# Tamnemng/TAM-GCN

Hardware: AMD Instinct MI355X
Metric: skeleton clips/sec (fwd+CE+bwd+grad all-reduce+SGD step), N-UCLA 20-joint x 64-frame (higher is better)
Workload: dtype f32 (exact fp32-input MFMA v_mfma_f32_16x16x4_f32 in every GEMM, forward and backward: the reference's arithmetic); 1 GPU; N-UCLA joint stream, 256 clips/GPU x (3,64,20,1), models.ctrgcn.Model fwd+CE+bwd+grad-allreduce+SGD step, train-mode BN; global_batch=256, streams=1, parallelism=dp1, launch=hipgraph, model_streams=0, rehearsal=False, allreduce=one flat bucket after backward

## Files before the change

include/tamgcn.h:

```cpp
#ifndef TAMGCN_H
#define TAMGCN_H

#ifdef __cplusplus
extern "C" {
#endif

#define TAMGCN_VERSION 401
#define TAMGCN_MAX_SUBSETS 3
#define TAMGCN_MAX_V 32

typedef struct tamgcn_src {
    const float* x1;
    const float* x2;
    const float* coef;
    int ctot;
    int coff;
    int act;
} tamgcn_src;

int         tamgcn_version(void);
const char* tamgcn_last_error(void);
const char* tamgcn_last_kernel(void);
int         tamgcn_get_split_mode(void);
int         tamgcn_set_split_mode(int mode);
// ... 86 lines not shown
    const float* pq;
    const float* w3;
    const float* b3;
    const float* w4;
    const float* b4;
    const float* A;
    const float* alpha;
    const float* E;
} tamgcn_ctrgc_desc;

int tamgcn_ctrgc_build_e(const tamgcn_ctrgc_desc* d, float* E, void* stream);

int tamgcn_ctrgc_fwd(const tamgcn_ctrgc_desc* d, float* y, float* stats_part, float* x3_out, void* stream);

int tamgcn_ctrgc_bwd_dx3(const tamgcn_ctrgc_desc* d, const tamgcn_src* dy,
                         float* dx3, float* db3_part, void* stream);

int tamgcn_ctrgc_bwd_de_acc(const tamgcn_ctrgc_desc* d, const tamgcn_src* dy, const float* x3,
                            float* dE, void* stream);
int tamgcn_ctrgc_bwd_de_tail(const tamgcn_ctrgc_desc* d, const float* dE,
                             float* dA_part, float* dw4_part, float* db4_part,
                             float* dalpha_part, float* dpq, int groups, void* stream);

int tamgcn_ctrgc_tiled_supported(int V);
int tamgcn_ctrgc_tiled_chunks(int V);
int tamgcn_ctrgc_tiled_build_e(const tamgcn_ctrgc_desc* d, float* E, void* stream);
int tamgcn_ctrgc_tiled_agg_fwd(const tamgcn_ctrgc_desc* d, const float* x3, const float* E, float* y, float* stats_part, void* stream);
int tamgcn_ctrgc_tiled_agg_bwd(const tamgcn_ctrgc_desc* d, const tamgcn_src* dy, const float* E, float* dx3, float* db3_part, void* stream);
int tamgcn_ctrgc_tiled_de_acc(const tamgcn_ctrgc_desc* d, const tamgcn_src* dy, const float* x3, float* dE, void* stream);
int tamgcn_ctrgc_tiled_de_tail(const tamgcn_ctrgc_desc* d, const float* dE, float* dA_part, float* dw4_part, float* db4_part,
                               float* dalpha_part, float* dpq, void* stream);

int tamgcn_vgen_supported(int V);
int tamgcn_vgen_lds_bytes(int S, int V, int R);
int tamgcn_vgen_build_e(const tamgcn_ctrgc_desc* d, float* E, void* stream);
int tamgcn_vgen_agg_fwd(const tamgcn_ctrgc_desc* d, const float* x3, const float* E, float* y, float* stats_part, void* stream);
int tamgcn_vgen_agg_bwd(const tamgcn_ctrgc_desc* d, const tamgcn_src* dy, const float* E, float* dx3, float* db3_part, void* stream);
int tamgcn_vgen_de_acc(const tamgcn_ctrgc_desc* d, const tamgcn_src* dy, const float* x3, float* dE, void* stream);
int tamgcn_vgen_de_tail(const tamgcn_ctrgc_desc* d, const float* dE, float* dA_part, float* dw4_part, float* db4_part,
                        float* dalpha_part, float* dpq, int groups, void* stream);

int tamgcn_ew_nparts(int N, int C, int T, int V);

int tamgcn_gcn_tail_fwd(const tamgcn_src* y, const tamgcn_src* o, const tamgcn_src* res,
                        int N, int C, int T, int V, float* g, void* stream);
int tamgcn_gcn_tail_bwd(const float* dg, const float* g, const tamgcn_src* o, const float* o_save,
// ... 156 lines not shown
```

tam_gcn_amd/_lib.py:

```python
import ctypes as C
import os

_HERE = os.path.dirname(os.path.abspath(__file__))
LIB_PATH = os.path.join(_HERE, 'libtamgcn.so')

c_float_p = C.c_void_p


class Src(C.Structure):
    _fields_ = [('x1', C.c_void_p), ('x2', C.c_void_p), ('coef', C.c_void_p),
                ('ctot', C.c_int), ('coff', C.c_int), ('act', C.c_int)]


class ConvDesc(C.Structure):
    _fields_ = [('src', Src),
                ('N', C.c_int), ('K', C.c_int), ('T_in', C.c_int), ('V', C.c_int),
                ('w', C.c_void_p), ('bias', C.c_void_p),
                ('M', C.c_int), ('KT', C.c_int), ('dil', C.c_int), ('stride', C.c_int), ('pad', C.c_int),
                ('wmode', C.c_int), ('up', C.c_int),
                ('y', C.c_void_p), ('yctot', C.c_int), ('ycoff', C.c_int),
                ('T_out', C.c_int), ('T_y', C.c_int), ('ostride', C.c_int),
                ('add1', C.c_void_p), ('add2', C.c_void_p), ('bcast', C.c_void_p), ('bcast_scale', C.c_float),
                ('mask', C.POINTER(Src)),
                ('aux', C.c_void_p), ('aux_center', C.c_void_p), ('auxctot', C.c_int), ('auxcoff', C.c_int),
# ... 91 lines not shown
    'tamgcn_conv_nparts': (_i, [C.POINTER(ConvDesc)]),
    'tamgcn_conv': (_i, [C.POINTER(ConvDesc), _p]),
    'tamgcn_wgrad_max_split': (_i, [C.POINTER(WgradDesc)]),
    'tamgcn_wgrad': (_i, [C.POINTER(WgradDesc), _p]),
    'tamgcn_stem_stats': (_i, [_p, _p, _p, _i, _i, _i, _i, _i, _p, _p]),
    'tamgcn_stem_apply': (_i, [_p, _p, _p, _i, _i, _i, _i, _i, _p, _p]),
    'tamgcn_head_pool_fwd': (_i, [_p, _i, _i, _i, _i, _i, _p, _p]),
    'tamgcn_head_pool_bwd': (_i, [_p, _i, _i, _i, _i, _i, _p, _p]),
    'tamgcn_head_fc_fwd': (_i, [_p, _p, _p, _i, _i, _i, _p, _p]),
    'tamgcn_head_fc_bwd': (_i, [_p, _p, _p, _i, _i, _i, _p, _p, _p, _p]),
    'tamgcn_reduce_multi': (_i, [C.POINTER(ReduceDesc), _i, _p]),
    'tamgcn_reduce_sum': (_i, [_p, _i, _ll, _ll, _f, _i, _p, _p]),
    'tamgcn_bn_fwd_finalize': (_i, [_p, _i, _i, _i, _d, _p, _p, _p, _p, _p, _f, _f, _i, _p, _p, _i, _i, _i, _p]),
    'tamgcn_bn_bwd_finalize': (_i, [_p, _i, _i, _i, _d, _p, _p, _i, _i, _i, _p, _p, _p, _p, _i, _i, _i, _p]),
    'tamgcn_bn_fwd_finalize_multi': (_i, [C.POINTER(BnFwdDesc), _i, _p]),
    'tamgcn_coef_diff': (_i, [_p, _p, _p, _i, _i, _p]),
    'tamgcn_bn_bwd_finalize_multi': (_i, [C.POINTER(BnBwdDesc), _i, _p]),
    'tamgcn_tmean': (_i, [_SP, _i, _i, _i, _i, _p, _p]),
    'tamgcn_ctrgc_build_e': (_i, [C.POINTER(CtrgcDesc), _p, _p]),
    'tamgcn_ctrgc_fwd': (_i, [C.POINTER(CtrgcDesc), _p, _p, _p, _p]),
    'tamgcn_ctrgc_bwd_dx3': (_i, [C.POINTER(CtrgcDesc), _SP, _p, _p, _p]),
    'tamgcn_ctrgc_bwd_de_acc': (_i, [C.POINTER(CtrgcDesc), _SP, _p, _p, _p]),
    'tamgcn_ctrgc_bwd_de_tail': (_i, [C.POINTER(CtrgcDesc), _p, _p, _p, _p, _p, _p, _i, _p]),
    'tamgcn_ctrgc_tiled_supported': (_i, [_i]),
    'tamgcn_ctrgc_tiled_chunks': (_i, [_i]),
    'tamgcn_ctrgc_tiled_build_e': (_i, [C.POINTER(CtrgcDesc), _p, _p]),
    'tamgcn_ctrgc_tiled_agg_fwd': (_i, [C.POINTER(CtrgcDesc), _p, _p, _p, _p, _p]),
    'tamgcn_ctrgc_tiled_agg_bwd': (_i, [C.POINTER(CtrgcDesc), _SP, _p, _p, _p, _p]),
    'tamgcn_ctrgc_tiled_de_acc': (_i, [C.POINTER(CtrgcDesc), _SP, _p, _p, _p]),
    'tamgcn_ctrgc_tiled_de_tail': (_i, [C.POINTER(CtrgcDesc), _p, _p, _p, _p, _p, _p, _p]),
    'tamgcn_vgen_supported': (_i, [_i]),
    'tamgcn_vgen_lds_bytes': (_i, [_i, _i, _i]),
    'tamgcn_vgen_build_e': (_i, [C.POINTER(CtrgcDesc), _p, _p]),
    'tamgcn_vgen_agg_fwd': (_i, [C.POINTER(CtrgcDesc), _p, _p, _p, _p, _p]),
    'tamgcn_vgen_agg_bwd': (_i, [C.POINTER(CtrgcDesc), _SP, _p, _p, _p, _p]),
    'tamgcn_vgen_de_acc': (_i, [C.POINTER(CtrgcDesc), _SP, _p, _p, _p]),
    'tamgcn_vgen_de_tail': (_i, [C.POINTER(CtrgcDesc), _p, _p, _p, _p, _p, _p, _i, _p]),
    'tamgcn_ew_nparts': (_i, [_i, _i, _i, _i]),
    'tamgcn_gcn_tail_fwd': (_i, [_SP, _SP, _SP, _i, _i, _i, _i, _p, _p]),
    'tamgcn_gcn_tail_bwd': (_i, [_p, _p, _SP, _p, _i, _i, _i, _i, _p, _p, _p, _p]),
    'tamgcn_gcn_mid_bwd': (_i, [_p, _p, _p, _p, _p, _p, _i, _i, _i, _i, _p, _p, _p, _p]),
    'tamgcn_tconv_supported': (_i, [_i, _i, _i, _i, C.POINTER(C.c_int), _i, _i]),
    'tamgcn_tconv_nparts': (_i, [C.POINTER(TconvDesc), _i]),
    'tamgcn_tconv_fwd': (_i, [C.POINTER(TconvDesc), _p]),
    'tamgcn_tconv_bwd': (_i, [C.POINTER(TconvDesc), _p]),
    'tamgcn_tconv_wgrad_max_split': (_i, [C.POINTER(TconvDesc)]),
# ... 79 lines not shown
```

tam_gcn_amd/build.py:

```python
import os
import subprocess
import sys

HERE = os.path.dirname(os.path.abspath(__file__))
SRC = ['lib.hip', 'conv.hip', 'wgrad.hip', 'reduce.hip', 'bn.hip', 'elementwise.hip', 'ctrgc.hip', 'ctrgc_de.hip', 'ctrgc_tiled.hip', 'vgen.hip', 'stemhead.hip', 'feeder.hip', 'f2.hip', 'f2v.hip', 'tconv.hip', 'optim.hip', 'evalmeter.hip']
LIB = os.path.join(HERE, 'libtamgcn.so')
ARCH = 'gfx950'


def _hipcc():
    for c in (os.environ.get('HIPCC'), '/opt/rocm/bin/hipcc', 'hipcc'):
        if c and (os.path.isabs(c) and os.path.exists(c) or not os.path.isabs(c)):
            return c
    return 'hipcc'


def sources():
    return [os.path.join(HERE, 'csrc', s) for s in SRC]


def needs_build():
    if not os.path.exists(LIB):
        return True
    deps = sources() + [os.path.join(HERE, 'csrc', 'common.h'), os.path.join(HERE, 'csrc', 'evalbody.h'),
                        os.path.join(HERE, '..', 'include', 'tamgcn.h')]
    t = os.path.getmtime(LIB)
    return any(os.path.getmtime(d) > t for d in deps)

# ... 28 lines not shown
```

tam_gcn_amd/csrc/ctrgc.hip:

```cpp
#include "common.h"
#include <stdlib.h>

TG_TRACE_DEFINE(tamgcn_trace_read_ctrgc)

#ifndef TG_CKO
#define TG_CKO 0
#endif

namespace {

struct CtrgcArgs {
    int N, Cin, Cout, S, T;
    const float* x; int x_ctot, x_coff;
    const float* w3; const float* b3;
    const float* E;
    int nct;
};

template <int V_, int CT_, int TB_, int NTQ_, int SBK_>
struct Geo {
    static constexpr int V = V_, CT = CT_, TB = TB_, NTQ = NTQ_, SBK = SBK_;
    static constexpr int SBKP = SBK + 2;
    static constexpr int NT = CT * NTQ * 4;
    static constexpr int NW = NT / 64;
// ... 143 lines not shown
                for (int k = 0; k < 8; ++k)
                    if (k * 4 < a.R) acc = mfma16(aw[k], Ds[(k * 4 + kq) * VV + colc], acc);
                if (col < VV) {
#pragma unroll
                    for (int r = 0; r < 4; ++r) Eg[(long long)(c0 + kq * 4 + r) * VV + col] = alpha * (acc[r] + b4r[r]) + Ar[it];
                }
            }
        }
        if (c0 + 16 < a.Cout) {
#pragma unroll
            for (int k = 0; k < 8; ++k) aw[k] = awn[k];
#pragma unroll
            for (int r = 0; r < 4; ++r) b4r[r] = b4n[r];
        }
    }
}

template <class G, int ST, bool UL = false>
struct X3Pref {
    using P = Plan<G, ST>;
    static constexpr int NPF = G::NPF, NT = G::NT, SBK = G::SBK, CT = G::CT;
    static constexpr int ROWV = G::NCOLS / 4;
    static constexpr int NAF = (P::NRT * 16 * SBK + NT - 1) / NT;
    float4 rv[NPF];
    float wv[NAF];

    __device__ __forceinline__ void load(const CtrgcArgs& a, int n, int c0, int t0, int bt, int k0, int tid) {
        if (TG_CKO & 2) return;
        constexpr int V = G::V;
        const int ncols = bt * V;
        const int cs = a.T * V;
        const float* xk = a.x + ((long long)n * a.x_ctot + a.x_coff + k0) * cs + (long long)t0 * V;
        const float* wk = a.w3 + (long long)c0 * a.Cin + k0;
        if constexpr (UL) {
            xk = a.x + cg_sgpr(((long long)n * a.x_ctot + a.x_coff + k0) * cs + (long long)t0 * V);
            wk = a.w3 + cg_sgpr((long long)c0 * a.Cin + k0);
        }
#pragma unroll
        for (int i = 0; i < NAF; ++i) {
            const int e = tid + i * NT;
            const int kk = e % SBK, row = e / SBK;
            const int sidx = row / CT, c = row - sidx * CT;
            const bool ok = row < P::NR && k0 + kk < a.Cin;
            if constexpr (UL) wv[i] = *cg_at<float>(wk, ok ? 4u * (unsigned)((sidx * a.Cout + c) * a.Cin + kk) : 0u);
            else wv[i] = ok ? *cg_at<float>(wk, 4u * (unsigned)((sidx * a.Cout + c) * a.Cin + kk)) : 0.f;
        }
#pragma unroll
        for (int i = 0; i < NPF; ++i) {
            const int e = tid + i * NT;
            const int kk = e / ROWV, pos = (e - kk * ROWV) * 4;
            const bool ok = kk < SBK && k0 + kk < a.Cin && pos < ncols;
            if constexpr (UL) rv[i] = *cg_at<float4>(xk, ok ? 4u * (unsigned)(kk * cs + pos) : 0u);
            else rv[i] = ok ? *cg_at<float4>(xk, 4u * (unsigned)(kk * cs + pos)) : make_float4(0.f, 0.f, 0.f, 0.f);
        }
    }
    __device__ __forceinline__ void pin() {
#pragma unroll
        for (int i = 0; i < NPF; ++i) asm volatile("" : "+v"(rv[i].x), "+v"(rv[i].y), "+v"(rv[i].z), "+v"(rv[i].w));
#pragma unroll
        for (int i = 0; i < NAF; ++i) asm volatile("" : "+v"(wv[i]));
    }
    __device__ __forceinline__ void commit(float* As, float* Bs, int tid, int Cin, int k0, int ncols) const {
        if (TG_CKO & 4) return;
#pragma unroll
        for (int i = 0; i < NAF; ++i) {
            const int e = tid + i * NT;
            const int kk = e % SBK, row = e / SBK;
            if constexpr (UL) {
                if (row < P::NRT * 16) As[row * G::SBKP + kk] = (row < P::NR && k0 + kk < Cin) ? wv[i] : 0.f;
            } else {
                if (row < P::NRT * 16) As[row * G::SBKP + kk] = wv[i];
            }
        }
#pragma unroll
        for (int i = 0; i < NPF; ++i) {
            const int e = tid + i * NT;
            const int kk = e / ROWV, pos = (e - kk * ROWV) * 4;
            if constexpr (UL) {
                if (kk < SBK) *reinterpret_cast<float4*>(Bs + kk * G::PITCHB + pos) = (k0 + kk < Cin && pos < ncols) ? rv[i] : make_float4(0.f, 0.f, 0.f, 0.f);
            } else {
                if (kk < SBK) *reinterpret_cast<float4*>(Bs + kk * G::PITCHB + pos) = rv[i];
            }
        }
    }
};

template <class G, int ST, bool UL, class Pre>
__device__ __forceinline__ void x3_chunk(const CtrgcArgs& a, int n, int c0, int t0, int bt, float* X3, X3Pref<G, ST, UL>& pf, int next_t0, int next_bt, int tid, Pre&& pre, float* B3s = nullptr, float b3v = 0.f) {
    using P = Plan<G, ST>;
    constexpr int V = G::V, CW = G::CW, SBK = G::SBK, SBKP = G::SBKP, CT = G::CT;
    constexpr int NR = P::NR, NRT = P::NRT, PB = G::PITCHB;
    const int lane = tid & 63, wave = tid >> 6;
    const int j = lane & 15, kq = lane >> 4;
    const int ncols = bt * V;
    constexpr bool BAL = (G::NW == 8 && G::NCT == 20);
    const int cw0 = BAL ? 5 * (wave & 3) + (wave < 4 ? 0 : 3) : wave * CW;
    const bool third = !BAL || wave < 4;
    float* Bs = X3;
    float* As = X3 + SBK * PB;

    f32x4 acc[NRT][CW];
#pragma unroll
// ... 36 lines not shown
#pragma unroll
                for (int rt = 0; rt < NRT; ++rt) asm volatile("" : "=v"(av[rt]));
#pragma unroll
                for (int c = 0; c < CW; ++c) asm volatile("" : "=v"(bv[c]));
            } else {
#pragma unroll
            for (int rt = 0; rt < NRT; ++rt) av[rt] = at[rt * 16 * SBKP + k4 * 4];
#pragma unroll
            for (int c = 0; c < CW; ++c) bv[c] = bt_[k4 * 4 * PB + bcol[c]];
            }
            if ((TG_CKO & 1) && k4) continue;
#pragma unroll
            for (int c = 0; c < (BAL ? 2 : CW); ++c)
#pragma unroll
                for (int rt = 0; rt < NRT; ++rt) acc[rt][c] = mfma16(av[rt], bv[c], acc[rt][c]);
            if (BAL && third) {
#pragma unroll
                for (int rt = 0; rt < NRT; ++rt) acc[rt][2] = mfma16(av[rt], bv[2], acc[rt][2]);
            }
        }
    }
    pre();
    __syncthreads();
#pragma unroll
    for (int rt = 0; rt < NRT; ++rt) {
        if constexpr (UL) {
            const f32x4 b = *reinterpret_cast<const f32x4*>(B3s + rt * 16 + kq * 4);
#pragma unroll
            for (int r = 0; r < 4; ++r) b3r[rt][r] = b[r];
        }
#pragma unroll
        for (int c = 0; c < CW; ++c) {
            int col = (cw0 + c) * 16 + j;
            if ((TG_CKO & 8) && (rt || c)) continue;
            if (col >= ncols || (BAL && c == 2 && !third)) continue;
            const int fr = col / V, v = col - fr * V;
#pragma unroll
            for (int r = 0; r < 4; ++r) {
                const int row = rt * 16 + kq * 4 + r;
                const int sidx = row / CT, ch = row - sidx * CT;
                if (row < NR) X3[(ch * G::BT + fr) * (ST * V) + sidx * V + v] = acc[rt][c][r] + b3r[rt][r];
            }
        }
    }
    __syncthreads();
}
// ... 195 lines not shown
        const int lrow = tid % (G::NTQ * 4);
        TG_T(ta);
        EFrag<G, ST> ef;
        x3_chunk<G, ST, !ER>(a, n, c0, t0, bt, X3, pf, nt0, nbt, tid, [&] { if constexpr (!ER) ef.ld(En, a.Cout, c0 + __builtin_amdgcn_readfirstlane(tid >> 6), tid); }, Zs, b3v);
        TG_T(tb); TG_ACC(1, tb - ta);
        if constexpr (!ER) aggregate_mfma_g<G, ST>(En, a.Cout, c0, ef, X3, Zs, bt, tid);
        else if (!(TG_CKO & 16)) aggregate_mfma<G, ST>(Es, X3, Zs, bt);
        TG_T(tc); TG_ACC(2, tc - tb);
        __syncthreads();
        TG_T(td); TG_ACC(3, td - tc);
        constexpr int RL = G::NTQ * 4;
        constexpr int NV4 = (G::NCOLS / 4 + RL - 1) / RL;
        float* ybase = y + (((long long)n * a.Cout + c0) * a.T + t0) * V;
        const unsigned rowb = 4u * (unsigned)(c * a.T * V);
        float4 zv[NV4];
#pragma unroll
        for (int i = 0; i < NV4; ++i) {
            const int p4 = lrow + i * RL;
            zv[i] = p4 < (ncols >> 2) ? reinterpret_cast<const float4*>(Zs + c * G::NCOLS)[p4] : make_float4(0.f, 0.f, 0.f, 0.f);
        }
        if (nbt > 0) pf.pin();
        if constexpr (!ER) {
            if (x3_out) {
#pragma unroll
                for (int s = 0; s < ST; ++s) {
                    float4 xs[NV4];
#pragma unroll
                    for (int i = 0; i < NV4; ++i) {
                        const int p4 = lrow + i * RL;
                        const int fr = p4 / (V / 4), q = p4 - fr * (V / 4);
                        xs[i] = p4 < (ncols >> 2) ? *reinterpret_cast<const float4*>(X3 + (c * G::BT + fr) * (ST * V) + s * V + 4 * q)
                                                  : make_float4(0.f, 0.f, 0.f, 0.f);
                    }
                    float* xo = x3_out + (((long long)n * ST * a.Cout + s * a.Cout + c0) * a.T + t0) * V;
#pragma unroll
                    for (int i = 0; i < NV4; ++i) {
                        const int p4 = lrow + i * RL;
                        if (p4 < (ncols >> 2)) *cg_at_w<float4>(xo, rowb + 16u * (unsigned)p4) = xs[i];
                    }
                }
            }
        } else
        if (x3_out) {
            float4 xv[ST][NV4];
#pragma unroll
            for (int s = 0; s < ST; ++s)
#pragma unroll
                for (int i = 0; i < NV4; ++i) {
                    const int p4 = lrow + i * RL;
                    const int fr = p4 / (V / 4), q = p4 - fr * (V / 4);
                    xv[s][i] = p4 < (ncols >> 2) ? *reinterpret_cast<const float4*>(X3 + (c * G::BT + fr) * (ST * V) + s * V + 4 * q)
                                                 : make_float4(0.f, 0.f, 0.f, 0.f);
                }
#pragma unroll
            for (int s = 0; s < ST; ++s) {
// ... 460 lines not shown
```

tam_gcn_amd/functional.py:

```python
import contextlib
import os
import threading

import torch

from . import ops
from .ops import S, RELU


_SIDE = {}
_SIDE_LOCK = threading.Lock()
USE_SIDE_STREAMS = os.environ.get('TAMGCN_SIDE_STREAMS', '1') != '0'

def _side_streams(device, main, k):
    key = (device.index, main.cuda_stream, k)
    got = _SIDE.get(key)
    if got is None:
        with _SIDE_LOCK:
            got = _SIDE.get(key)
            if got is None:
                taken = {main.cuda_stream}
                for (d, m, _), ss in _SIDE.items():
                    if d == device.index:
                        taken.add(m)
# ... 174 lines not shown
    ev = None
    if EVAL_FUSED and not training and not save:
        bns = [P.bn, P.bno] + ([P.bnd] if P.mode == 'conv' else [])

        def build():
            cy, sy = _eval_coefs([(P.bn, 0)], Cout, x)
            co, so = _eval_coefs([(P.bno, 0)], Cout, x)
            cd, sd_ = _eval_coefs([(P.bnd, 0)], Cout, x) if P.mode == 'conv' else (None, None)
            cdiff = ops.coef_diff(cd, cy, {'conv': 0, 'identity': 1}.get(P.mode, 2))
            return dict(y=(cy, sy), o=(co, so), d=(cd, sd_), diff=cdiff)
        ev = _eval_cached(P.bn.m, 'unit_gcn', bns, build)
    if P.mode == 'conv':
        with fk.on(0):
            d_pre, dpart = ops.conv(xs, K=Cin, w=P.Wd, bias=P.bd, M=Cout, stats=training)
            if ev is not None:
                coef_d, save_d = ev['d']
    xbar = taken_xbar(x, Cin)
    if xbar is None:
        xbar = ops.tmean(xs, Cin)
    pq, _ = ops.conv(S(xbar.view(1, Cin, N, V)), K=Cin, w=P.W12, bias=P.B12, M=S_ * 2 * R)
    pq = pq.view(S_ * 2 * R, N, V)
    E = ops.ctrgc_build_E(xs, pq, P.W3, P.B3, P.W4, P.B4, P.PA, P.alpha, Cin, Cout, S_, R)
    y_pre, ypart, x3 = ops.ctrgc_fwd(xs, pq, P.W3, P.B3, P.W4, P.B4, P.PA, P.alpha, Cin, Cout, S_, R, stats=training,
                                     keep_x3=save, E=E)
    fk.__exit__()
    if ev is not None:
        coef_y, save_y = ev['y']
    else:
        bb = ops.BNBatch()
        coef_y, save_y = _coef(Cout, x)
        P.bn.fwd(ypart, 0, count, training, coef_y, save_y, 0, batch=bb)
        if P.mode == 'conv':
            coef_d, save_d = _coef(Cout, x)
            P.bnd.fwd(dpart, 0, count, training, coef_d, save_d, 0, batch=bb)
        bb.flush()
    if P.mode == 'conv':
        res = S(d_pre, coef=coef_d)
        coef_diff = ev['diff'] if ev is not None else ops.coef_diff(coef_d, coef_y, 0)
        diff = S(d_pre, y_pre, coef_diff)
    elif P.mode == 'identity':
        res = xs
        coef_diff = ev['diff'] if ev is not None else ops.coef_diff(None, coef_y, 1)
        diff = S(x, y_pre, coef_diff)
    else:
        res = None
        coef_diff = ev['diff'] if ev is not None else ops.coef_diff(None, coef_y, 2)
        diff = S(y_pre, None, coef_diff)
# ... 417 lines not shown
        dg, dxres, Gt = tcn_backward(ctx.Pt, ctx.svt, dout.contiguous(), need_dg=True, need_dxres=need_dx)
        ctx.svt = None
        dx, Gg = gcn_backward(ctx.Pg, ctx.svg, dg, need_dx=need_dx, extra_dx=dxres)
        ctx.svg = None
        return (None, dx, None, None) + tuple(ctx.mod.gcn1._route(Gg)) + tuple(ctx.mod._route_tcn(Gt))


class CTRGCFn(_Fn):
    @staticmethod
    def forward(ctx, x, A, alpha, w1, b1, w2, b2, w3, b3, w4, b4):
        N, Cin, T, V = x.shape
        Cout, R = w3.shape[0], w1.shape[0]
        W12 = torch.cat((w1.reshape(R, Cin), w2.reshape(R, Cin)))
        B12 = torch.cat((b1, b2))
        W3, W4 = w3.reshape(Cout, Cin), w4.reshape(1, Cout, R)
        A3 = A.reshape(1, V, V).contiguous()
        al = alpha.reshape(1).to(torch.float32).contiguous()
        xs = S(x)
        xbar = ops.tmean(xs, Cin)
        pq, _ = ops.conv(S(xbar.view(1, Cin, N, V)), K=Cin, w=W12, bias=B12, M=2 * R)
        pq = pq.view(2 * R, N, V)
        save = _needs(ctx)
        E = ops.ctrgc_build_E(xs, pq, W3, b3, W4, b4.reshape(1, Cout), A3, al, Cin, Cout, 1, R)
        y, _, x3 = ops.ctrgc_fwd(xs, pq, W3, b3, W4, b4.reshape(1, Cout), A3, al, Cin, Cout, 1, R, stats=False, keep_x3=save, E=E)
        ctx.sv = (x, xbar, pq, W12, W3, b3, W4, b4.reshape(1, Cout), A3, al, E, x3) if save else None
        ctx.shapes = (A.shape, alpha.shape, w1.shape, w3.shape, w4.shape)
        return y

    @staticmethod
    def backward(ctx, dy):
        x, xbar, pq, W12, W3, b3, W4, b4, A3, al, E, x3 = ctx.sv
        ctx.sv = None
        N, Cin, T, V = x.shape
        Cout, R = W3.shape[0], W4.shape[2]
        xs = S(x)
        dx3, db3, dA, dW4, db4, dal, dpq = ops.ctrgc_bwd(xs, pq, W3, b3, W4, b4, A3, al, Cin, Cout, 1, R,
                                                         S(dy.contiguous()), x3=x3, E=E)
        dpq4 = S(dpq.view(1, 2 * R, N, V))
        dW12 = ops.wgrad(dpq4, S(xbar.view(1, Cin, N, V)), M=2 * R, K=Cin)
        dB12 = dpq.sum((1, 2))
        dW3 = ops.wgrad(S(dx3), xs, M=Cout, K=Cin)
        dx = None
        if ctx.needs_input_grad[0]:
            dxbar, _ = ops.conv(dpq4, K=2 * R, w=W12, bias=None, M=Cin, wmode=1)
            dx, _ = ops.conv(S(dx3), K=Cout, w=W3, bias=None, M=Cin, wmode=1, bcast=dxbar.view(Cin, N, V),
                             bcast_scale=1.0 / T)
        As, als, w1s, w3s, w4s = ctx.shapes
# ... 122 lines not shown
    K, V = Ae.shape[0], Ae.shape[1]
    N = x.shape[0]
    dev = x.device
    R = 4
    z = torch.zeros
    return dict(pq=z(K * 2 * R, N, V, device=dev), w4=z(K, Cout, R, device=dev), b4=z(K, Cout, device=dev),
                A=Ae.transpose(1, 2).contiguous(), alpha=z(1, device=dev), R=R, K=K)


class StGcnFn(_Fn):

    @staticmethod
    def forward(ctx, mod, tail, x, Ae, w3, b3, g1, be1, wt, bt, g2, be2, *res_params):
        N, Cin, T, V = x.shape
        Cout, s, kt = mod.out_channels, mod.stride, mod.t_kernel
        training = mod.training
        save = _needs(ctx)
        bn1, bn2 = BN(mod.tcn[0]), BN(mod.tcn[3])
        xs = S(x)
        W3, Ae = w3.reshape(w3.shape[0], Cin), Ae.contiguous()
        a = _stgcn_ctrgc_args(x, Ae, W3, b3, Cout)
        cargs = (xs, a['pq'], W3, b3, a['w4'], a['b4'], a['A'], a['alpha'], Cin, Cout, a['K'], a['R'])
        E = ops.ctrgc_build_E(*cargs)
        y_pre, ypart, x3 = ops.ctrgc_fwd(*cargs, stats=training, keep_x3=save, E=E)
        cnt1 = N * T * V
        coef1, save1 = _coef(Cout, x)
        bn1.fwd(ypart, 0, cnt1, training, coef1, save1, 0)
        pad = (kt - 1) // 2
        z_pre, zpart = ops.conv(S(y_pre, coef=coef1, act=RELU), K=Cout, w=wt, bias=bt, M=Cout, KT=kt, stride=s, pad=pad, stats=training)
        T2 = z_pre.shape[2]
        cnt2 = N * T2 * V
        coef2, save2 = _coef(Cout, x)
        bn2.fwd(zpart, 0, cnt2, training, coef2, save2, 0)
        r_pre = coef_r = save_r = None
        rmode = mod._rmode if tail else 'zero'
        if rmode == 'identity':
            res = xs
        elif rmode == 'conv':
            wr, br = res_params[0], res_params[1]
            bnr = BN(mod.residual[1])
            r_pre, rpart = ops.conv(xs, K=Cin, w=wr, bias=br, M=Cout, KT=1, stride=s, pad=0, T_out=T2, stats=training)
            coef_r, save_r = _coef(Cout, x)
            bnr.fwd(rpart, 0, cnt2, training, coef_r, save_r, 0)
            res = S(r_pre, coef=coef_r)
        else:
            res = None
        out = ops.add_act_fwd(S(z_pre, coef=coef2), res, bool(tail), Cout)
# ... 119 lines not shown
```

tam_gcn_amd/ops.py:

```python
import ctypes as C
import os
import threading

import torch

from . import _lib
from ._lib import Src, ConvDesc, WgradDesc, CtrgcDesc, ReduceDesc, TconvDesc, TCONV_MAXB

RELU = 1


def _stream():
    return C.c_void_p(torch.cuda.current_stream().cuda_stream)


def _ptr(t):
    if t is None:
        return None
    if not (t.is_cuda and t.is_contiguous()):
        raise RuntimeError('tam_gcn_amd: expected a contiguous HIP (cuda) tensor; there is no CPU path')
    if t.dtype not in (torch.float32, torch.int64, torch.int32, torch.float64):
        raise RuntimeError(f'tam_gcn_amd: unsupported dtype {t.dtype}')
    return t.data_ptr()

# ... 484 lines not shown
        _lib.check(_lib_().tamgcn_ctrgc_bwd_dx3(C.byref(d), C.byref(dyc), _ptr(dx3), _ptr(db3_part), _stream()),
                   'tamgcn_ctrgc_bwd_dx3')
    return dx3, (reduce_sum(db3_part, N, chunks=[(Cout,)] * S) if per_subset else reduce_sum(db3_part, N))


def ctrgc_bwd_de_acc(dy, x3, Cout, S):
    N, _, T, V = x3.shape
    d = CtrgcDesc()
    d.N, d.Cout, d.S, d.T, d.V = N, Cout, S, T, V
    dE = empty(N, S, Cout, V, V, like=x3)
    if ctrgc_route(V) != 'fused':
        acc, name = _agg_entry(V, 'de_acc')
        for n0, n1 in n_chunks(N, S * Cout * T * V):
            d.N = n1 - n0
            dyc = _slice_src(dy, n0, n1).c()
            _lib.check(acc(C.byref(d), C.byref(dyc), _ptr(x3[n0:n1]), _ptr(dE[n0:n1]), _stream()), name)
    else:
        dyc = dy.c()
        _lib.check(_lib_().tamgcn_ctrgc_bwd_de_acc(C.byref(d), C.byref(dyc), _ptr(x3), _ptr(dE), _stream()),
                   'tamgcn_ctrgc_bwd_de_acc')
    return dE


def ctrgc_bwd_de_tail(dE, pq, w4, b4, alpha, R, per_subset=False, groups=1):
    N, S, Cout, V, _ = dE.shape
    d = CtrgcDesc()
    d.N, d.Cout, d.S, d.R, d.V = N, Cout, S, R, V
    d.pq, d.w4, d.b4, d.alpha = _ptr(pq), _ptr(w4), _ptr(b4), _ptr(alpha)
    like = dE
    ps = per_subset
    if ctrgc_route(V) == 'tiled':
        if groups != 1:
            raise RuntimeError('tam_gcn_amd: the tiled dE tail (V in {32, 64}) has no channel groups')
        NUC = _lib_().tamgcn_ctrgc_tiled_chunks(V)
        dA_part = empty(N, S, V, V, like=like)
        dw4_part = empty(N * NUC, S, Cout, R, like=like)
        db4_part = empty(N * NUC, S, Cout, like=like)
        dal_part = empty(N * S * NUC, 1, like=like)
        dpq = empty(NUC, S * 2 * R, N, V, like=like)
        _lib.check(_lib_().tamgcn_ctrgc_tiled_de_tail(C.byref(d), _ptr(dE), _ptr(dA_part), _ptr(dw4_part), _ptr(db4_part), _ptr(dal_part),
                                                      _ptr(dpq), _stream()), 'tamgcn_ctrgc_tiled_de_tail')
        return (reduce_sum(dA_part, N), reduce_sum(dw4_part, N * NUC, chunks=[(Cout, R, 1, 1)] * S if ps else None),
                reduce_sum(db4_part, N * NUC, chunks=[(Cout,)] * S if ps else None), reduce_sum(dal_part, N * S * NUC),
                reduce_sum(dpq, NUC, immediate=True))
    if R > 32:
        raise RuntimeError('tam_gcn_amd: CTRGC with R > 32 rel-channels is not built')
    G = groups
    dA_part = empty(N * G, S, V, V, like=like)
    dw4_part = empty(N, S, Cout, R, like=like)
    db4_part = empty(N, S, Cout, like=like)
    dal_part = empty(N * S * G, 1, like=like)
    dpq = empty(G, S * 2 * R, N, V, like=like)
    name = 'tamgcn_vgen_de_tail' if ctrgc_route(V) == 'vgen' else 'tamgcn_ctrgc_bwd_de_tail'
    _lib.check(getattr(_lib_(), name)(C.byref(d), _ptr(dE), _ptr(dA_part), _ptr(dw4_part), _ptr(db4_part),
                                      _ptr(dal_part), _ptr(dpq), G, _stream()), name)
    dpq = dpq[0] if G == 1 else reduce_sum(dpq, G, immediate=True)
    return (reduce_sum(dA_part, N * G), reduce_sum(dw4_part, N, chunks=[(Cout, R, 1, 1)] * S if ps else None),
            reduce_sum(db4_part, N, chunks=[(Cout,)] * S if ps else None), reduce_sum(dal_part, N * S * G), dpq)


def ctrgc_bwd_de(x, pq, w3, b3, w4, b4, A, alpha, Cin, Cout, S, R, dy, x3=None, per_subset=False):
    if x3 is None:
        x3 = _x3_gemm(x, w3, b3, Cin, Cout, S)
    dE = ctrgc_bwd_de_acc(dy, x3, Cout, S)
    return ctrgc_bwd_de_tail(dE, pq, w4, b4, alpha, R, per_subset=per_subset)


def ctrgc_bwd(x, pq, w3, b3, w4, b4, A, alpha, Cin, Cout, S, R, dy, x3=None, E=None):
    dx3, db3 = ctrgc_bwd_dx3(x, pq, w3, b3, w4, b4, A, alpha, Cin, Cout, S, R, dy, E=E)
    dA, dw4, db4, dal, dpq = ctrgc_bwd_de(x, pq, w3, b3, w4, b4, A, alpha, Cin, Cout, S, R, dy, x3)
    return dx3, db3, dA, dw4, db4, dal, dpq


def gcn_tail_fwd(y, o, res):
    N, _, T, V = y.x1.shape
    Cc = y.ctot
    g = empty(N, Cc, T, V, like=y.x1)
    yc, oc = y.c(), o.c()
    rc = res.c() if res is not None else None
    _lib.check(_lib_().tamgcn_gcn_tail_fwd(C.byref(yc), C.byref(oc), C.byref(rc) if rc is not None else None,
                                           N, Cc, T, V, _ptr(g), _stream()), 'tamgcn_gcn_tail_fwd')
    return g


def gcn_tail_bwd(dg, g, o, o_save):
    N, Cc, T, V = g.shape
    dsum, doz = empty_like(g), empty_like(g)
# ... 328 lines not shown
```

Before: 9196 clips/s.

## Recompute CTRGC x3 inside the dE accumulation kernel for small-Cin layers

For CTRGC layers with small input channel count (Cin ≤ 4, e.g. the first layer with 3 input channels), the forward pass no longer stores the large x3 activation (S·Cout·T·V). A new fused backward kernel rebuilds x3 on the fly with a single MFMA step from x, w3 and b3 into LDS, then accumulates dE from dy. This removes the x3 store in forward and its reload in backward, in exchange for some recompute inside the kernel. The change also removes some integer index arithmetic (unsigned div/mod, guards dropped when tiles are full) in the CTRGC GEMM loader and the x3 store path.

Result: no change. 9256 clips/s (median of 2 runs) (+0.6%).

```diff
diff --git a/include/tamgcn.h b/include/tamgcn.h
--- a/include/tamgcn.h
+++ b/include/tamgcn.h
@@ -132,6 +132,8 @@
                              float* dA_part, float* dw4_part, float* db4_part,
                              float* dalpha_part, float* dpq, int groups, void* stream);
 
+int tamgcn_ctrgc_bwd_de_acc_x(const tamgcn_ctrgc_desc* d, const tamgcn_src* dy, float* dE, void* stream);
+
 int tamgcn_ctrgc_tiled_supported(int V);
 int tamgcn_ctrgc_tiled_chunks(int V);
 int tamgcn_ctrgc_tiled_build_e(const tamgcn_ctrgc_desc* d, float* E, void* stream);
diff --git a/tam_gcn_amd/_lib.py b/tam_gcn_amd/_lib.py
--- a/tam_gcn_amd/_lib.py
+++ b/tam_gcn_amd/_lib.py
@@ -137,6 +137,7 @@
     'tamgcn_ctrgc_bwd_dx3': (_i, [C.POINTER(CtrgcDesc), _SP, _p, _p, _p]),
     'tamgcn_ctrgc_bwd_de_acc': (_i, [C.POINTER(CtrgcDesc), _SP, _p, _p, _p]),
     'tamgcn_ctrgc_bwd_de_tail': (_i, [C.POINTER(CtrgcDesc), _p, _p, _p, _p, _p, _p, _i, _p]),
+    'tamgcn_ctrgc_bwd_de_acc_x': (_i, [C.POINTER(CtrgcDesc), _SP, _p, _p]),
     'tamgcn_ctrgc_tiled_supported': (_i, [_i]),
     'tamgcn_ctrgc_tiled_chunks': (_i, [_i]),
     'tamgcn_ctrgc_tiled_build_e': (_i, [C.POINTER(CtrgcDesc), _p, _p]),
diff --git a/tam_gcn_amd/build.py b/tam_gcn_amd/build.py
--- a/tam_gcn_amd/build.py
+++ b/tam_gcn_amd/build.py
@@ -3,7 +3,7 @@
 import sys
 
 HERE = os.path.dirname(os.path.abspath(__file__))
-SRC = ['lib.hip', 'conv.hip', 'wgrad.hip', 'reduce.hip', 'bn.hip', 'elementwise.hip', 'ctrgc.hip', 'ctrgc_de.hip', 'ctrgc_tiled.hip', 'vgen.hip', 'stemhead.hip', 'feeder.hip', 'f2.hip', 'f2v.hip', 'tconv.hip', 'optim.hip', 'evalmeter.hip']
+SRC = ['lib.hip', 'conv.hip', 'wgrad.hip', 'reduce.hip', 'bn.hip', 'elementwise.hip', 'ctrgc.hip', 'ctrgc_de.hip', 'ctrgc_de_x.hip', 'ctrgc_tiled.hip', 'vgen.hip', 'stemhead.hip', 'feeder.hip', 'f2.hip', 'f2v.hip', 'tconv.hip', 'optim.hip', 'evalmeter.hip']
 LIB = os.path.join(HERE, 'libtamgcn.so')
 ARCH = 'gfx950'
 
diff --git a/tam_gcn_amd/csrc/ctrgc.hip b/tam_gcn_amd/csrc/ctrgc.hip
--- a/tam_gcn_amd/csrc/ctrgc.hip
+++ b/tam_gcn_amd/csrc/ctrgc.hip
@@ -1,5 +1,6 @@
 #include "common.h"
 #include <stdlib.h>
+#include <type_traits>
 
 TG_TRACE_DEFINE(tamgcn_trace_read_ctrgc)
 
@@ -189,6 +190,10 @@
     static constexpr int NPF = G::NPF, NT = G::NT, SBK = G::SBK, CT = G::CT;
     static constexpr int ROWV = G::NCOLS / 4;
     static constexpr int NAF = (P::NRT * 16 * SBK + NT - 1) / NT;
+    using IT = typename std::conditional<UL, unsigned, int>::type;
+    static constexpr bool AFULL = UL && P::NRT * 16 * SBK == NAF * NT;
+    static constexpr bool ANR = AFULL && P::NR == P::NRT * 16;
+    static constexpr bool BFULL = UL && SBK * ROWV == NPF * NT;
     float4 rv[NPF];
     float wv[NAF];
 
@@ -205,18 +210,18 @@
         }
 #pragma unroll
         for (int i = 0; i < NAF; ++i) {
-            const int e = tid + i * NT;
-            const int kk = e % SBK, row = e / SBK;
-            const int sidx = row / CT, c = row - sidx * CT;
+            const IT e = (IT)tid + i * NT;
+            const int kk = (int)(e % SBK), row = (int)(e / SBK);
+            const int sidx = (int)((IT)row / CT), c = row - sidx * CT;
             const bool ok = row < P::NR && k0 + kk < a.Cin;
             if constexpr (UL) wv[i] = *cg_at<float>(wk, ok ? 4u * (unsigned)((sidx * a.Cout + c) * a.Cin + kk) : 0u);
             else wv[i] = ok ? *cg_at<float>(wk, 4u * (unsigned)((sidx * a.Cout + c) * a.Cin + kk)) : 0.f;
         }
 #pragma unroll
         for (int i = 0; i < NPF; ++i) {
-            const int e = tid + i * NT;
-            const int kk = e / ROWV, pos = (e - kk * ROWV) * 4;
-            const bool ok = kk < SBK && k0 + kk < a.Cin && pos < ncols;
+            const IT e = (IT)tid + i * NT;
+            const int kk = (int)(e / ROWV), pos = ((int)e - kk * ROWV) * 4;
+            const bool ok = (BFULL || kk < SBK) && k0 + kk < a.Cin && pos < ncols;
             if constexpr (UL) rv[i] = *cg_at<float4>(xk, ok ? 4u * (unsigned)(kk * cs + pos) : 0u);
             else rv[i] = ok ? *cg_at<float4>(xk, 4u * (unsigned)(kk * cs + pos)) : make_float4(0.f, 0.f, 0.f, 0.f);
         }
@@ -231,20 +236,20 @@
         if (TG_CKO & 4) return;
 #pragma unroll
         for (int i = 0; i < NAF; ++i) {
-            const int e = tid + i * NT;
-            const int kk = e % SBK, row = e / SBK;
+            const IT e = (IT)tid + i * NT;
+            const int kk = (int)(e % SBK), row = (int)(e / SBK);
             if constexpr (UL) {
-                if (row < P::NRT * 16) As[row * G::SBKP + kk] = (row < P::NR && k0 + kk < Cin) ? wv[i] : 0.f;
+                if (AFULL || row < P::NRT * 16) As[row * G::SBKP + kk] = ((ANR || row < P::NR) && k0 + kk < Cin) ? wv[i] : 0.f;
             } else {
                 if (row < P::NRT * 16) As[row * G::SBKP + kk] = wv[i];
             }
         }
 #pragma unroll
         for (int i = 0; i < NPF; ++i) {
-            const int e = tid + i * NT;
-            const int kk = e / ROWV, pos = (e - kk * ROWV) * 4;
+            const IT e = (IT)tid + i * NT;
+            const int kk = (int)(e / ROWV), pos = ((int)e - kk * ROWV) * 4;
             if constexpr (UL) {
-                if (kk < SBK) *reinterpret_cast<float4*>(Bs + kk * G::PITCHB + pos) = (k0 + kk < Cin && pos < ncols) ? rv[i] : make_float4(0.f, 0.f, 0.f, 0.f);
+                if (BFULL || kk < SBK) *reinterpret_cast<float4*>(Bs + kk * G::PITCHB + pos) = (k0 + kk < Cin && pos < ncols) ? rv[i] : make_float4(0.f, 0.f, 0.f, 0.f);
             } else {
                 if (kk < SBK) *reinterpret_cast<float4*>(Bs + kk * G::PITCHB + pos) = rv[i];
             }
@@ -327,6 +332,26 @@
     }
     pre();
     __syncthreads();
+    if constexpr (UL && NR == NRT * 16 && CT == 16) {
+        int xo[CW];
+#pragma unroll
+        for (int c = 0; c < CW; ++c) {
+            const int col = (cw0 + c) * 16 + j;
+            const int fr = col / V;
+            xo[c] = (kq * 4 * G::BT + fr) * (ST * V) + (col - fr * V);
+        }
+#pragma unroll
+        for (int rt = 0; rt < NRT; ++rt) {
+            const f32x4 b = *reinterpret_cast<const f32x4*>(B3s + rt * 16 + kq * 4);
+#pragma unroll
+            for (int c = 0; c < CW; ++c) {
+                if ((TG_CKO & 8) && (rt || c)) continue;
+                if ((cw0 + c) * 16 + j >= ncols || (BAL && c == 2 && !third)) continue;
+#pragma unroll
+                for (int r = 0; r < 4; ++r) X3[xo[c] + r * G::BT * (ST * V) + rt * V] = acc[rt][c][r] + b[r];
+            }
+        }
+    } else
 #pragma unroll
     for (int rt = 0; rt < NRT; ++rt) {
         if constexpr (UL) {
@@ -568,15 +593,20 @@
         if (nbt > 0) pf.pin();
         if constexpr (!ER) {
             if (x3_out) {
+                int xr[NV4];
+#pragma unroll
+                for (int i = 0; i < NV4; ++i) {
+                    const int p4 = lrow + i * RL;
+                    const int fr = p4 / (V / 4);
+                    xr[i] = (c * G::BT + fr) * (ST * V) + 4 * (p4 - fr * (V / 4));
+                }
 #pragma unroll
                 for (int s = 0; s < ST; ++s) {
                     float4 xs[NV4];
 #pragma unroll
                     for (int i = 0; i < NV4; ++i) {
                         const int p4 = lrow + i * RL;
-                        const int fr = p4 / (V / 4), q = p4 - fr * (V / 4);
-                        xs[i] = p4 < (ncols >> 2) ? *reinterpret_cast<const float4*>(X3 + (c * G::BT + fr) * (ST * V) + s * V + 4 * q)
-                                                  : make_float4(0.f, 0.f, 0.f, 0.f);
+                        xs[i] = p4 < (ncols >> 2) ? *reinterpret_cast<const float4*>(X3 + xr[i] + s * V) : make_float4(0.f, 0.f, 0.f, 0.f);
                     }
                     float* xo = x3_out + (((long long)n * ST * a.Cout + s * a.Cout + c0) * a.T + t0) * V;
 #pragma unroll
diff --git a/tam_gcn_amd/csrc/ctrgc_de_x.hip b/tam_gcn_amd/csrc/ctrgc_de_x.hip
--- /dev/null
+++ b/tam_gcn_amd/csrc/ctrgc_de_x.hip
@@ -0,0 +1,191 @@
+#include "common.h"
+
+namespace {
+
+template <int ST_>
+struct AccXGeo {
+    static constexpr int V = 20, ST = ST_, VV = V * V;
+    static constexpr int CA = 8;
+    static constexpr int NT = 256, NW = NT / 64;
+    static constexpr int BT = 16;
+    static constexpr int NCOLS = BT * V;
+    static constexpr int PX = NCOLS + 4;
+    static constexpr int PZ = NCOLS + 20;
+    static constexpr int NUG0 = (NT / (ST * CA)) < V ? (NT / (ST * CA)) : V;
+    static constexpr int UBG = (V + NUG0 - 1) / NUG0;
+    static constexpr int NUG = (V + UBG - 1) / UBG;
+    static constexpr int NOWN = ST * CA * NUG;
+    static constexpr int ROWV = NCOLS / 4;
+    static constexpr int NY = (CA * ROWV + NT - 1) / NT;
+    static constexpr int NR = ST * CA;
+    static constexpr int NRT = (NR + 15) / 16;
+    static constexpr int NCT = NCOLS / 16;
+    static constexpr int CW = NCT / NW;
+    static constexpr size_t LDS = sizeof(float) * (size_t)(ST * CA * PX + CA * PZ);
+    static_assert(NOWN <= NT, "not enough threads for the dE owners");
+    static_assert(NCOLS % 16 == 0 && NCT % NW == 0, "whole column tiles, the same number per wave");
+};
+
+struct AccXArgs {
+    int N, Cin, Cout, T;
+    const float* x; int x_ctot, x_coff;
+    const float* w3; const float* b3;
+};
+
+template <class G>
+__global__ __launch_bounds__(G::NT) void ctrgc_de_acc_x_kernel(const AccXArgs a, const SrcDev dy, float* __restrict__ dE) {
+    constexpr int V = G::V, VV = G::VV, ST = G::ST, NT = G::NT, CA = G::CA, UBG = G::UBG, NRT = G::NRT, CW = G::CW;
+    extern __shared__ __attribute__((aligned(16))) float smem[];
+    float* X3 = smem;
+    float* Zs = smem + ST * CA * G::PX;
+    const int nca = a.Cout / CA;
+    const int n = blockIdx.x / nca, c0 = (blockIdx.x - n * nca) * CA;
+    const int tid = threadIdx.x, lane = tid & 63, wave = tid >> 6, j = lane & 15, kq = lane >> 4;
+    const int own_s = tid / (CA * G::NUG), own_c = (tid / G::NUG) % CA, own_g = tid % G::NUG;
+    const bool owner = tid < G::NOWN;
+    const long long cs = (long long)a.T * V;
+
+    float aw[NRT], b3r[NRT][4];
+#pragma unroll
+    for (int rt = 0; rt < NRT; ++rt) {
+        const int row = rt * 16 + j;
+        aw[rt] = (row < G::NR && kq < a.Cin) ? a.w3[(long long)((row / CA) * a.Cout + c0 + row % CA) * a.Cin + kq] : 0.f;
+#pragma unroll
+        for (int r = 0; r < 4; ++r) {
+            const int orow = rt * 16 + kq * 4 + r;
+            b3r[rt][r] = orow < G::NR ? a.b3[(orow / CA) * a.Cout + c0 + orow % CA] : 0.f;
+        }
+    }
+    const float* xk = a.x + ((long long)n * a.x_ctot + a.x_coff + (kq < a.Cin ? kq : 0)) * cs;
+
+    float xb[CW], y1[G::NY][4], y2[G::NY][4], k1[G::NY], k2[G::NY], k0[G::NY];
+    auto load = [&](int t0, int bt) {
+        const int ncols = bt * V;
+#pragma unroll
+        for (int i = 0; i < CW; ++i) {
+            const int col = (wave * CW + i) * 16 + j;
+            xb[i] = (kq < a.Cin && col < ncols) ? xk[(long long)t0 * V + col] : 0.f;
+        }
+#pragma unroll
+        for (int i = 0; i < G::NY; ++i) {
+            int e = tid + i * NT;
+            int row = e / G::ROWV, pos = (e - row * G::ROWV) * 4;
+            bool ok = row < CA && pos < ncols;
+            int ch = dy.coff + c0 + (ok ? row : 0);
+            long long g = ((long long)n * dy.ctot + ch) * cs + (long long)t0 * V + (ok ? pos : 0);
+            k1[i] = dy.coef ? dy.coef[ch] : 1.f;
+            k2[i] = (dy.coef && dy.x2) ? dy.coef[dy.ctot + ch] : 0.f;
+            k0[i] = dy.coef ? dy.coef[2 * dy.ctot + ch] : 0.f;
+            float4 t = ok ? *reinterpret_cast<const float4*>(dy.x1 + g) : make_float4(0.f, 0.f, 0.f, 0.f);
+            float4 u = (ok && dy.x2) ? *reinterpret_cast<const float4*>(dy.x2 + g) : make_float4(0.f, 0.f, 0.f, 0.f);
+            y1[i][0] = t.x; y1[i][1] = t.y; y1[i][2] = t.z; y1[i][3] = t.w;
+            y2[i][0] = u.x; y2[i][1] = u.y; y2[i][2] = u.z; y2[i][3] = u.w;
+        }
+    };
+    auto commit = [&]() {
+#pragma unroll
+        for (int rt = 0; rt < NRT; ++rt)
+#pragma unroll
+            for (int i = 0; i < CW; ++i) {
+                f32x4 acc = mfma16(aw[rt], xb[i], (f32x4){0.f, 0.f, 0.f, 0.f});
+                acc = mfma16(0.f, 0.f, acc);
+                const int col = (wave * CW + i) * 16 + j;
+#pragma unroll
+                for (int r = 0; r < 4; ++r) {
+                    const int orow = rt * 16 + kq * 4 + r;
+                    if (orow < G::NR) X3[orow * G::PX + col] = acc[r] + b3r[rt][r];
+                }
+            }
+#pragma unroll
+        for (int i = 0; i < G::NY; ++i) {
+            int e = tid + i * NT;
+            int row = e / G::ROWV, pos = (e - row * G::ROWV) * 4;
+            if (row < CA) {
+                float o[4];
+#pragma unroll
+                for (int k = 0; k < 4; ++k) {
+                    float v = fmaf(k1[i], y1[i][k], fmaf(k2[i], y2[i][k], k0[i]));
+                    o[k] = dy.act == 1 ? fmaxf(v, 0.f) : v;
+                }
+                *reinterpret_cast<float4*>(Zs + row * G::PZ + pos) = make_float4(o[0], o[1], o[2], o[3]);
+            }
+        }
+    };
+
+    float acc[UBG][V];
+#pragma unroll
+    for (int i = 0; i < UBG; ++i)
+#pragma unroll
+        for (int v = 0; v < V; ++v) acc[i][v] = 0.f;
+
+    for (int t0 = 0; t0 < a.T; t0 += G::BT) {
+        const int bt = min(G::BT, a.T - t0);
+        load(t0, bt);
+        __syncthreads();
+        commit();
+        __syncthreads();
+        if (owner) {
+            const float* xr = X3 + (own_s * CA + own_c) * G::PX;
+            const float* dr = Zs + own_c * G::PZ + own_g * UBG;
+            for (int tl = 0; tl < bt; ++tl) {
+                float xv[V], d[UBG];
+#pragma unroll
+                for (int v = 0; v < V; v += 4) {
+                    f32x4 t = *reinterpret_cast<const f32x4*>(xr + tl * V + v);
+                    xv[v] = t[0]; xv[v + 1] = t[1]; xv[v + 2] = t[2]; xv[v + 3] = t[3];
+                }
+                if constexpr (UBG == 2) {
+                    float2 t = *reinterpret_cast<const float2*>(dr + tl * V);
+                    d[0] = t.x; d[1] = t.y;
+                } else {
+#pragma unroll
+                    for (int i = 0; i < UBG; ++i) d[i] = (own_g * UBG + i < V) ? dr[tl * V + i] : 0.f;
+                }
+#pragma unroll
+                for (int i = 0; i < UBG; ++i)
+#pragma unroll
+                    for (int v = 0; v < V; ++v) acc[i][v] = fmaf(d[i], xv[v], acc[i][v]);
+            }
+        }
+    }
+    if (owner) {
+        float* o = dE + (((long long)n * ST + own_s) * a.Cout + c0 + own_c) * VV;
+#pragma unroll
+        for (int i = 0; i < UBG; ++i) {
+            const int u = own_g * UBG + i;
+            if (u < V) {
+#pragma unroll
+                for (int v = 0; v < V; v += 4)
+                    *reinterpret_cast<float4*>(o + u * V + v) = make_float4(acc[i][v], acc[i][v + 1], acc[i][v + 2], acc[i][v + 3]);
+            }
+        }
+    }
+}
+
+template <class G>
+void launch_acc_x(const AccXArgs& a, const tamgcn_src* dy, float* dE, void* stream) {
+    tg_launch_lds<ctrgc_de_acc_x_kernel<G>>(G::LDS, dim3(a.N * (a.Cout / G::CA)), dim3(G::NT), G::LDS, (hipStream_t)stream, a, make_src(*dy), dE);
+    tamgcn_note_kernel("ctrgc_de_acc_x_kernel<AccXGeo<%d>>", G::ST);
+}
+
+}
+
+extern "C" int tamgcn_ctrgc_bwd_de_acc_x(const tamgcn_ctrgc_desc* d, const tamgcn_src* dy, float* dE, void* stream) {
+    TG_CHECK(d && dy && dy->x1 && dE, "tamgcn_ctrgc_bwd_de_acc_x: null pointer");
+    TG_CHECK(d->x.x1 && d->w3 && d->b3, "tamgcn_ctrgc_bwd_de_acc_x: null x / w3 / b3 (x3 is rebuilt from them)");
+    TG_CHECK(d->N > 0 && d->T > 0 && d->Cout > 0 && d->Cout % 8 == 0, "tamgcn_ctrgc_bwd_de_acc_x: bad shape N=%d T=%d Cout=%d", d->N, d->T, d->Cout);
+    TG_CHECK(d->Cin >= 1 && d->Cin <= 4 && (d->S == 1 || d->S == 3) && d->V == 20,
+             "tamgcn_ctrgc_bwd_de_acc_x: unsupported Cin=%d S=%d V=%d (1 <= Cin <= 4, S in {1,3}, V = 20; otherwise keep x3: tamgcn_ctrgc_bwd_de_acc)", d->Cin, d->S, d->V);
+    TG_CHECK(!(d->x.x2 || d->x.coef || d->x.act), "tamgcn_ctrgc_bwd_de_acc_x: x must be a plain tensor (no fused prologue)");
+    TG_CHECK(d->x.coff >= 0 && d->x.coff + d->Cin <= d->x.ctot, "tamgcn_ctrgc_bwd_de_acc_x: x channel slice out of range");
+    TG_CHECK(dy->coff >= 0 && dy->ctot >= dy->coff + d->Cout, "tamgcn_ctrgc_bwd_de_acc_x: dy has %d channels from %d, need %d", dy->ctot, dy->coff, d->Cout);
+    TG_CHECK((long long)d->N * (d->Cout / 8) < (1LL << 31), "tamgcn_ctrgc_bwd_de_acc_x: N * Cout / 8 >= 2^31 workgroups");
+    AccXArgs a;
+    a.N = d->N; a.Cin = d->Cin; a.Cout = d->Cout; a.T = d->T;
+    a.x = d->x.x1; a.x_ctot = d->x.ctot; a.x_coff = d->x.coff;
+    a.w3 = d->w3; a.b3 = d->b3;
+    if (d->S == 3) launch_acc_x<AccXGeo<3>>(a, dy, dE, stream);
+    else launch_acc_x<AccXGeo<1>>(a, dy, dE, stream);
+    TG_LAUNCH_CHECK("tamgcn_ctrgc_bwd_de_acc_x");
+    return 0;
+}
diff --git a/tam_gcn_amd/functional.py b/tam_gcn_amd/functional.py
--- a/tam_gcn_amd/functional.py
+++ b/tam_gcn_amd/functional.py
@@ -220,7 +220,7 @@
     pq = pq.view(S_ * 2 * R, N, V)
     E = ops.ctrgc_build_E(xs, pq, P.W3, P.B3, P.W4, P.B4, P.PA, P.alpha, Cin, Cout, S_, R)
     y_pre, ypart, x3 = ops.ctrgc_fwd(xs, pq, P.W3, P.B3, P.W4, P.B4, P.PA, P.alpha, Cin, Cout, S_, R, stats=training,
-                                     keep_x3=save, E=E)
+                                     keep_x3=save and not ops.ctrgc_recomputes_x3(Cin, S_, V), E=E)
     fk.__exit__()
     if ev is not None:
         coef_y, save_y = ev['y']
@@ -684,7 +684,8 @@
         pq = pq.view(2 * R, N, V)
         save = _needs(ctx)
         E = ops.ctrgc_build_E(xs, pq, W3, b3, W4, b4.reshape(1, Cout), A3, al, Cin, Cout, 1, R)
-        y, _, x3 = ops.ctrgc_fwd(xs, pq, W3, b3, W4, b4.reshape(1, Cout), A3, al, Cin, Cout, 1, R, stats=False, keep_x3=save, E=E)
+        y, _, x3 = ops.ctrgc_fwd(xs, pq, W3, b3, W4, b4.reshape(1, Cout), A3, al, Cin, Cout, 1, R, stats=False,
+                                 keep_x3=save and not ops.ctrgc_recomputes_x3(Cin, 1, V), E=E)
         ctx.sv = (x, xbar, pq, W12, W3, b3, W4, b4.reshape(1, Cout), A3, al, E, x3) if save else None
         ctx.shapes = (A.shape, alpha.shape, w1.shape, w3.shape, w4.shape)
         return y
@@ -853,7 +854,7 @@
         a = _stgcn_ctrgc_args(x, Ae, W3, b3, Cout)
         cargs = (xs, a['pq'], W3, b3, a['w4'], a['b4'], a['A'], a['alpha'], Cin, Cout, a['K'], a['R'])
         E = ops.ctrgc_build_E(*cargs)
-        y_pre, ypart, x3 = ops.ctrgc_fwd(*cargs, stats=training, keep_x3=save, E=E)
+        y_pre, ypart, x3 = ops.ctrgc_fwd(*cargs, stats=training, keep_x3=save and not ops.ctrgc_recomputes_x3(Cin, a['K'], V), E=E)
         cnt1 = N * T * V
         coef1, save1 = _coef(Cout, x)
         bn1.fwd(ypart, 0, cnt1, training, coef1, save1, 0)
diff --git a/tam_gcn_amd/ops.py b/tam_gcn_amd/ops.py
--- a/tam_gcn_amd/ops.py
+++ b/tam_gcn_amd/ops.py
@@ -530,6 +530,25 @@
     return dE
 
 
+X3_RECOMPUTE_MAX_CIN = 4
+
+
+def ctrgc_recomputes_x3(Cin, S, V):
+    return 1 <= Cin <= X3_RECOMPUTE_MAX_CIN and S in (1, 3) and ctrgc_route(V) == 'fused'
+
+
+def ctrgc_bwd_de_acc_x(x, w3, b3, Cin, Cout, S, dy):
+    N, _, T, V = x.x1.shape
+    d = CtrgcDesc()
+    d.N, d.Cin, d.Cout, d.S, d.T, d.V = N, Cin, Cout, S, T, V
+    d.x = x.c()
+    d.w3, d.b3 = _ptr(w3), _ptr(b3)
+    dE = empty(N, S, Cout, V, V, like=x.x1)
+    dyc = dy.c()
+    _lib.check(_lib_().tamgcn_ctrgc_bwd_de_acc_x(C.byref(d), C.byref(dyc), _ptr(dE), _stream()), 'tamgcn_ctrgc_bwd_de_acc_x')
+    return dE
+
+
 def ctrgc_bwd_de_tail(dE, pq, w4, b4, alpha, R, per_subset=False, groups=1):
     N, S, Cout, V, _ = dE.shape
     d = CtrgcDesc()
@@ -568,9 +587,12 @@
 
 
 def ctrgc_bwd_de(x, pq, w3, b3, w4, b4, A, alpha, Cin, Cout, S, R, dy, x3=None, per_subset=False):
-    if x3 is None:
-        x3 = _x3_gemm(x, w3, b3, Cin, Cout, S)
-    dE = ctrgc_bwd_de_acc(dy, x3, Cout, S)
+    if x3 is None and ctrgc_recomputes_x3(Cin, S, x.x1.shape[3]):
+        dE = ctrgc_bwd_de_acc_x(x, w3, b3, Cin, Cout, S, dy)
+    else:
+        if x3 is None:
+            x3 = _x3_gemm(x, w3, b3, Cin, Cout, S)
+        dE = ctrgc_bwd_de_acc(dy, x3, Cout, S)
     return ctrgc_bwd_de_tail(dE, pq, w4, b4, alpha, R, per_subset=per_subset)
 
 
```
